# nsirons/DL-unet

Measured on AMD Instinct MI355X. Metric: 572x572 tiles/sec fwd+bwd, higher is better.
Workload: dtype f32; 1 GPU; batch=8/GPU 572x572x1 fwd+bwd+SGD fp32, 64-base-ch U-Net (BASELINE configs[1]); arithmetic=fp32 MFMA; 3x3 fwd/dgrad/wgrad as Winograd F(2x2,3x3), global_batch=8, tile=572, parallelism=dp1, loss=unweighted BCE-with-logits

## Files before the change

dl-unet_amd/csrc/wgradw.hip:

```cpp
#include "common.hpp"
#include "kernel_parts.hpp"
#include <cstdio>
#include <cstdlib>

namespace unet {

struct WgradWK {
    WgradP p;
    int TXn, TXg, TYn;
    int wy0, wx0;
    int NTg;
    int nsteps, steps_per;
    int ntile_i, ntile_j, nsplit;
    FastDiv d_spi, d_txg;
    size_t pstride;
    int xbytes, ybytes;
};

#ifndef WW_DBG
#define WW_DBG 0
#endif
constexpr int WW_PATCH = 32768, WW_EXTRA = 2048, WW_DY = 16384;
constexpr int WW_STAGE = WW_PATCH + WW_EXTRA + WW_DY;
constexpr int WW_NST = 3;
constexpr int WW_LDS = WW_NST * WW_STAGE;
constexpr int WW_SLAB = 9 * 64 * 64 + 64;

template <int N> __device__ __forceinline__ void ww_wait_vmcnt() { asm volatile("s_waitcnt vmcnt(%0)" ::"n"(N) : "memory"); }

__device__ __forceinline__ f32x2 wpk_add(f32x2 a, f32x2 b) { return a + b; }
__device__ __forceinline__ f32x2 wpk_sub(f32x2 a, f32x2 b) { return a - b; }

template <bool BUF>
__global__ __launch_bounds__(512, 1) void wgradw_f32_kernel(const WgradWK k)
{
    const WgradP &p = k.p;
    extern __shared__ __attribute__((aligned(16))) unsigned char smem[];

    const int tid = threadIdx.x, lane = tid & 63;
    const int wave = __builtin_amdgcn_readfirstlane(tid >> 6);
    const int wi = wave >> 1, wj = wave & 1;
    const int l15 = lane & 15, kg = lane >> 4;

    const int logical = xcd_slot();
    const int ntile = k.ntile_i * k.ntile_j;
    const int part = logical / ntile, tile = logical - part * ntile;
    const int it = tile / k.ntile_j, jt = tile - it * k.ntile_j;
    const int s0 = part * k.steps_per;
    int s1 = s0 + k.steps_per;
    s1 = s1 < k.nsteps ? s1 : k.nsteps;
    const int ns = s1 > s0 ? s1 - s0 : 0;

    const int d_cb = wave & 3, d_par = (wave >> 2) & 1;
    const int spi = k.TYn * k.TXg;

    const __amdgpu_buffer_rsrc_t rs_x = make_rsrc(p.X, BUF ? k.xbytes : 0);
    const __amdgpu_buffer_rsrc_t rs_y = make_rsrc(p.Y, BUF ? k.ybytes : 0);
    auto stage = [&](int buf, int step) {
        unsigned char *sb = smem + buf * WW_STAGE;
        int ln = lane;
        asm volatile("" : "+v"(ln));
        const int d_slot = ln >> 2, d_chunk = ln & 3;
        const int xch = p.xc0 + it * 64 + d_cb * 16 + d_chunk * 4;
        const int ych = p.yc0 + jt * 64 + d_cb * 16 + d_chunk * 4;
        const int Tb = step * 16;
        const bool tok = Tb + d_slot < k.NTg;
        const int img_b = fdiv(Tb, k.d_spi);
        const int rem_b = Tb - img_b * spi;
        const int ty_b = fdiv(rem_b, k.d_txg);
        int img = img_b, ty = ty_b, txg = rem_b - ty_b * k.TXg + d_slot;
        while (txg >= k.TXg) { txg -= k.TXg; ++ty; }
        while (ty >= k.TYn) { ty -= k.TYn; ++img; }
        img = img < p.NB ? img : p.NB - 1;
        {
            const int iy0 = (k.wy0 + 2 * ty + p.oy0) - p.xpad, ix = (k.wx0 + 2 * txg + p.ox0) - p.xpad + d_par;
            const bool xok = tok && (unsigned)ix < (unsigned)p.XW;
            const int base = ((img * p.XH + iy0) * p.XW + ix) * p.XC + xch;
#pragma unroll
            for (int qy = 0; qy < 4; ++qy) {
                const bool ok = xok && (unsigned)(iy0 + qy) < (unsigned)p.XH;
                unsigned char *dst = sb + ((qy * 2 + d_par) * 4 + d_cb) * 1024;
                if (BUF) {
                    lds_dma16(rs_x, dst, ok ? (base + qy * p.XW * p.XC) * 4 : LDS_DMA_OOB, 0);
                } else {
                    const float *g = ok ? p.X + (base + qy * p.XW * p.XC) : p.zeros;
                    GLDS16(g, dst);
                }
            }
        }
        {
            const int yy0 = k.wy0 + 2 * ty, xx = k.wx0 + 2 * txg + d_par;
            const bool xok = tok && txg < k.TXn && xx < p.YW;
            const int base = ((img * p.YH + yy0) * p.YW + xx) * p.YC + ych;
#pragma unroll
            for (int py = 0; py < 2; ++py) {
                const bool ok = xok && yy0 + py < p.YH;
                unsigned char *dst = sb + WW_PATCH + WW_EXTRA + ((py * 2 + d_par) * 4 + d_cb) * 1024;
                if (BUF) {
                    lds_dma16(rs_y, dst, ok ? (base + py * p.YW * p.YC) * 4 : LDS_DMA_OOB, 0);
                } else {
                    const float *g = ok ? p.Y + (base + py * p.YW * p.YC) : p.zeros;
                    GLDS16(g, dst);
                }
            }
        }
        if (wave < 2) {
            const int Te = step * 16 + 16;
            const bool eok = Te < k.NTg;
            const int Tec = eok ? Te : k.NTg - 1;
            const int eimg = fdiv(Tec, k.d_spi);
            const int erem = Tec - eimg * spi;
            const int ety = fdiv(erem, k.d_txg);
            const int etxg = erem - ety * k.TXg;
            const int e_row = (ln >> 4) + 4 * wave, e_cb = (ln >> 2) & 3;
            const int e_xch = p.xc0 + it * 64 + e_cb * 16 + d_chunk * 4;
            const int qy = e_row >> 1, par = e_row & 1;
            const int iy = (k.wy0 + 2 * ety + p.oy0) - p.xpad + qy, ix = (k.wx0 + 2 * etxg + p.ox0) - p.xpad + par;
            const bool ok = eok && (unsigned)iy < (unsigned)p.XH && (unsigned)ix < (unsigned)p.XW;
            const int eoff = ((eimg * p.XH + iy) * p.XW + ix) * p.XC + e_xch;
            if (BUF) {
                lds_dma16(rs_x, sb + WW_PATCH + wave * 1024, ok ? eoff * 4 : LDS_DMA_OOB, 0);
            } else {
                const float *g = ok ? p.X + eoff : p.zeros;
                GLDS16(g, sb + WW_PATCH + wave * 1024);
            }
        }
    };
    auto wait_landed = [&](bool one_in_flight) {
        if (!one_in_flight) ww_wait_vmcnt<0>();
        else if (wave < 2) ww_wait_vmcnt<7>();
        else ww_wait_vmcnt<6>();
    };

    f32x4 acc[16][2];
#pragma unroll
    for (int x = 0; x < 16; ++x)
#pragma unroll
        for (int j = 0; j < 2; ++j)
#pragma unroll
            for (int r = 0; r < 4; ++r) acc[x][j][r] = 0.f;
    f32x2 dbacc[2] = {{0.f, 0.f}, {0.f, 0.f}};

    const int a_base = wi * 1024 + l15 * 4;
    const int e_base = WW_PATCH + wi * 64 + l15 * 4;
    const bool last = kg == 3;
    const int y_base = WW_PATCH + WW_EXTRA + l15 * 4;

#define WW_SB() __builtin_amdgcn_sched_barrier(0)
    const int lv = a_base + kg * 64;
    const int lx = last ? e_base : lv + 9 * 64 + 256;
    const int lxs = last ? 512 : 8192;
    const int ly = y_base + 2 * wj * 1024 + kg * 64;
    auto v_read = [&](int buf, int pr, int j, f32x2 (&a)[4]) {
        if (WW_DBG & 4) { WW_SB(); return; }
        const unsigned char *pv = smem + buf * WW_STAGE + lv;
        if (j < 2 || pr == 0) {
#pragma unroll
            for (int qy = 0; qy < 4; ++qy) {
                const unsigned char *src = pv + ((2 * qy + (j & 1)) * 4096 + (8 * pr + (j >> 1)) * 64);
                a[qy][0] = *(const float *)(src);
                a[qy][1] = *(const float *)(src + 256);
            }
        } else {
            const unsigned char *px = smem + buf * WW_STAGE + lx + (j & 1) * (lxs >> 1);
#pragma unroll
            for (int qy = 0; qy < 4; ++qy) {
                a[qy][0] = *(const float *)(pv + ((2 * qy + (j & 1)) * 4096 + 9 * 64));
                a[qy][1] = *(const float *)(px + qy * lxs);
            }
        }
        WW_SB();
    };
    auto v_col = [&](int j, const f32x2 (&a)[4], f32x2 (&v)[16]) {
        if (WW_DBG & 8) { WW_SB(); return; }
        v[j] = wpk_sub(a[0], a[2]);
        v[4 + j] = wpk_add(a[1], a[2]);
        v[8 + j] = wpk_sub(a[2], a[1]);
        v[12 + j] = wpk_sub(a[1], a[3]);
        WW_SB();
    };
    auto v_row = [&](int i, f32x2 (&v)[16]) {
        if (WW_DBG & 8) { WW_SB(); return; }
        const f32x2 t0 = v[4 * i], t1 = v[4 * i + 1], t2 = v[4 * i + 2], t3 = v[4 * i + 3];
        v[4 * i + 0] = wpk_sub(t0, t2);
        v[4 * i + 1] = wpk_add(t1, t2);
        v[4 * i + 2] = wpk_sub(t2, t1);
        v[4 * i + 3] = wpk_sub(t1, t3);
        WW_SB();
    };
    auto z_read = [&](int buf, int pr, int c, f32x2 (&d)[4]) {
        if (WW_DBG & 4) { WW_SB(); return; }
        const unsigned char *ys = smem + buf * WW_STAGE + ly;
#pragma unroll
        for (int px = 0; px < 4; ++px) {
            d[px][0] = *(const float *)(ys + (px * 4096 + c * 1024 + pr * 512));
            d[px][1] = *(const float *)(ys + (px * 4096 + c * 1024 + pr * 512 + 256));
        }
        WW_SB();
    };
    auto group = [&](const f32x2 (&v)[16], const f32x2 (&d)[4], int c, bool RD, bool XF, int bufz, int prz, int cz, f32x2 (&dn)[4],
                     int bufv, int prv, f32x2 (&r)[4][4], f32x2 (&vn)[16]) {
        f32x2 zt[4];
        auto quad = [&](int b, int h) {
#pragma unroll
            for (int e = 0; e < 4; ++e)
                acc[4 * b + e][c] = __builtin_amdgcn_mfma_f32_16x16x4f32(v[4 * b + e][h], zt[e][h], acc[4 * b + e][c], 0, 0, 0);
            WW_SB();
        };
        zt[0] = d[0]; zt[1] = wpk_add(d[0], d[1]); zt[2] = wpk_sub(d[0], d[1]); zt[3] = d[1];
        WW_SB();
        quad(0, 0);
        z_read(bufz, prz, cz, dn);
        quad(0, 1);
        if (RD) v_read(bufv, prv, 0, r[0]);
        if (XF) { v_col(0, r[0], vn); v_col(1, r[1], vn); }
        zt[0] = wpk_add(d[0], d[2]); zt[3] = wpk_add(d[1], d[3]); zt[1] = wpk_add(zt[0], zt[3]); zt[2] = wpk_sub(zt[0], zt[3]);
        WW_SB();
        quad(1, 0);
        if (RD) v_read(bufv, prv, 1, r[1]);
        if (XF) { v_col(2, r[2], vn); v_col(3, r[3], vn); }
        quad(1, 1);
        if (RD) v_read(bufv, prv, 2, r[2]);
        if (XF) v_row(0, vn);
        zt[0] = wpk_sub(d[0], d[2]); zt[3] = wpk_sub(d[1], d[3]); zt[1] = wpk_add(zt[0], zt[3]); zt[2] = wpk_sub(zt[0], zt[3]);
        WW_SB();
        quad(2, 0);
        if (RD) v_read(bufv, prv, 3, r[3]);
        if (XF) v_row(1, vn);
        quad(2, 1);
        if (XF) v_row(2, vn);
        zt[0] = d[2]; zt[1] = wpk_add(d[2], d[3]); zt[2] = wpk_sub(d[2], d[3]); zt[3] = d[3];
        dbacc[c] = wpk_add(dbacc[c], wpk_add(wpk_add(d[0], d[1]), zt[1]));
        WW_SB();
        quad(3, 0);
        if (XF) {
            v_row(3, vn);
#pragma unroll
            for (int i = 0; i < 16; ++i) asm volatile("" : "+v"(vn[i]));
        }
        quad(3, 1);
    };
    if (ns > 0) {
        stage(0, s0);
        if (ns > 1) stage(1, s0 + 1);
        wait_landed(ns > 1);
        __builtin_amdgcn_s_barrier();
        const bool early = wave < 4;
        f32x2 va[16], vb[16], da[4], db_[4], r[4][4];
        {
#pragma unroll
            for (int j = 0; j < 4; ++j) { v_read(0, 0, j, r[j]); v_col(j, r[j], va); }
#pragma unroll
            for (int i = 0; i < 4; ++i) v_row(i, va);
        }
        z_read(0, 0, 0, da);
        for (int s = 0; s < ns; ++s) {
            const bool more = s + 2 < ns;
            const int buf = s % WW_NST, nbuf = (s + 1) % WW_NST;
            WW_SB();
            group(va, da, 0, true, false, buf, 0, 1, db_, buf, 1, r, vb);
            group(va, db_, 1, false, true, buf, 1, 0, da, buf, 1, r, vb);
            if (!(WW_DBG & 1)) ww_wait_vmcnt<0>();
            if (!(WW_DBG & 2)) __builtin_amdgcn_s_barrier();
            WW_SB();
            if (more && early && !(WW_DBG & 1)) stage((s + 2) % WW_NST, s0 + s + 2);
            WW_SB();
            group(vb, da, 0, true, false, buf, 1, 1, db_, nbuf, 0, r, va);
            group(vb, db_, 1, false, true, nbuf, 0, 0, da, nbuf, 0, r, va);
            if (more && !early && !(WW_DBG & 1)) stage((s + 2) % WW_NST, s0 + s + 2);
            WW_SB();
        }
    }
#undef WW_SB

    float *slab = p.slab + (size_t)(tile * k.nsplit + part) * k.pstride;
#pragma unroll
    for (int c = 0; c < 2; ++c) {
        f32x4 r[3][4];
#pragma unroll
        for (int b = 0; b < 4; ++b) {
            const f32x4 m0 = b == 3 ? -acc[b][c] : acc[b][c];
            const f32x4 m1 = b == 3 ? -acc[4 + b][c] : acc[4 + b][c];
            const f32x4 m2 = b == 3 ? -acc[8 + b][c] : acc[8 + b][c];
            const f32x4 m3 = b == 3 ? acc[12 + b][c] : -acc[12 + b][c];
            const f32x4 h = 0.5f * (m1 + m2);
            r[0][b] = m0 + h;
            r[1][b] = 0.5f * (m1 - m2);
            r[2][b] = h + m3;
        }
#pragma unroll
        for (int a = 0; a < 3; ++a) {
            const f32x4 h = 0.5f * (r[a][1] + r[a][2]);
            const f32x4 o0 = r[a][0] + h, o1 = 0.5f * (r[a][1] - r[a][2]), o2 = h + r[a][3];
            float *dst = slab + ((a * 3) * 64 + (2 * wj + c) * 16 + l15) * 64 + wi * 16 + 4 * kg;
            *(f32x4 *)(dst) = o0;
            *(f32x4 *)(dst + 4096) = o1;
            *(f32x4 *)(dst + 8192) = o2;
        }
    }
    if (wi == 0) {
#pragma unroll
        for (int c = 0; c < 2; ++c) {
            float v = dbacc[c][0] + dbacc[c][1];
            v += __shfl_xor(v, 16, 64);
            v += __shfl_xor(v, 32, 64);
            if (kg == 0) slab[9 * 64 * 64 + (2 * wj + c) * 16 + l15] = v;
        }
    }
}

template <int PG>
__global__ __launch_bounds__(64 * PG) void wgradw_reduce_kernel(const float *__restrict__ slab, int nsplit, size_t pstride, int ntile_j,
                                                            float *__restrict__ out, long si, long sj, long st,
                                                            float *__restrict__ db, int db_c0)
{
    const int tile = blockIdx.x >> 6, jb = blockIdx.x & 63;
    const int j = threadIdx.x & 63, grp = threadIdx.x >> 6;
    const float *src = slab + (size_t)tile * nsplit * pstride + (size_t)jb * 64 + j;
    float m[9];
#pragma unroll
    for (int x = 0; x < 9; ++x) m[x] = 0.f;
    for (int P = grp; P < nsplit; P += PG) {
        const float *s = src + (size_t)P * pstride;
#pragma unroll
        for (int x = 0; x < 9; ++x) m[x] += s[x * 4096];
    }
    __shared__ float red[PG][3][64];
#pragma unroll
    for (int xq = 0; xq < 3; ++xq) {
        if (xq) __syncthreads();
#pragma unroll
        for (int x = 0; x < 3; ++x) red[grp][x][j] = m[3 * xq + x];
        __syncthreads();
        if (grp == 0) {
#pragma unroll
            for (int x = 0; x < 3; ++x) {
                float v = red[0][x][j];
#pragma unroll
                for (int g = 1; g < PG; ++g) v += red[g][x][j];
                m[3 * xq + x] = v;
            }
        }
    }
    if (grp == 0) {
        const int it = tile / ntile_j, jt = tile - it * ntile_j;
        float *o = out + (size_t)(it * 64 + j) * si + (size_t)(jt * 64 + jb) * sj;
#pragma unroll
        for (int t = 0; t < 9; ++t) o[t * st] = m[t];
    }
    if (db && jb == 0 && (tile / ntile_j) == 0) {
        __syncthreads();
        const int jt = tile % ntile_j;
        float v = 0.f;
        for (int P = grp; P < nsplit; P += PG) v += slab[((size_t)tile * nsplit + P) * pstride + 9 * 64 * 64 + j];
        red[grp][0][j] = v;
        __syncthreads();
        if (grp == 0) {
            float t = red[0][0][j];
#pragma unroll
            for (int g = 1; g < PG; ++g) t += red[g][0][j];
            db[db_c0 + jt * 64 + j] = t;
        }
    }
}

bool wgradw_applicable(const WgradP &p)
{
    if (p.TY != 3 || p.TX != 3 || p.stride != 1) return false;
    if (p.Ci % 64 != 0 || p.Cj % 64 != 0 || p.db_on_x) return false;
    return true;
}

static void ww_decompose(const WgradP &p, WgradWK &k, int cus)
{
    k.p = p;
    k.wy0 = p.ywin0; k.wx0 = p.xwin0;
    k.TYn = cdiv(p.ywin1 - p.ywin0, 2);
    k.TXn = cdiv(p.xwin1 - p.xwin0, 2);
    k.TXg = k.TXn + 1;
    k.NTg = p.NB * k.TYn * k.TXg;
    k.nsteps = cdiv(k.NTg, 16);
    k.ntile_i = p.Ci / 64; k.ntile_j = p.Cj / 64;
    const int ntile = k.ntile_i * k.ntile_j;
    int nsplit = cus / ntile;
    if (nsplit < 1) nsplit = 1;
    if (nsplit > k.nsteps) nsplit = k.nsteps;
    k.nsplit = nsplit;
    k.steps_per = cdiv(k.nsteps, nsplit);
    k.d_spi = make_fastdiv((unsigned)(k.TYn * k.TXg));
    k.d_txg = make_fastdiv((unsigned)k.TXg);
    k.pstride = WW_SLAB;
}

size_t wgradw_slab_need(const WgradP &p)
{
    if (!wgradw_applicable(p)) return 0;
    WgradWK k;
    ww_decompose(p, k, 256);
    return (size_t)k.ntile_i * k.ntile_j * k.nsplit * k.pstride * sizeof(float);
}

int launch_wgradw(const WgradP &p, hipStream_t st)
{
    const size_t xb = tensor_bytes(p.NB, p.XH, p.XW, p.XC, sizeof(float)), yb = tensor_bytes(p.NB, p.YH, p.YW, p.YC, sizeof(float));
    const bool buf = get_lds_dma_mode() != 0 && fits_buffer(xb) && fits_buffer(yb);
    const auto launch = buf ? launch_profiled<wgradw_f32_kernel<true>, WgradWK> : launch_profiled<wgradw_f32_kernel<false>, WgradWK>;
    WgradWK k;
    int cus = device_cu_count();
    if (cus > 256) cus = 256;
    ww_decompose(p, k, cus);
    k.xbytes = buf ? (int)xb : 0; k.ybytes = buf ? (int)yb : 0;
    const int ntile = k.ntile_i * k.ntile_j;
    const size_t need = (size_t)ntile * k.nsplit * k.pstride * sizeof(float);
    ARG_CHECK(need <= p.slab_bytes, "wgradw: slab scratch too small (%zu < %zu)", p.slab_bytes, need);
    ARG_CHECK(tensor_elems(p.NB, p.XH, p.XW, p.XC) < LIMIT_31BIT && tensor_elems(p.NB, p.YH, p.YW, p.YC) < LIMIT_31BIT,
              "wgradw: tensor exceeds 31-bit element offsets");
    if (p.db) ARG_CHECK(p.ywin0 == 0 && p.xwin0 == 0 && p.ywin1 == p.YH && p.xwin1 == p.YW, "wgradw: fused bias gradient needs the full Y window");
    char tag[96];
    snprintf(tag, sizeof(tag), "wgradw<%d> Ci=%d Cj=%d Y=%dx%d tiles=%dx%d steps=%d split=%d", (int)buf, p.Ci, p.Cj, p.YH, p.YW, k.TYn, k.TXn, k.nsteps, k.nsplit);
    if (int rc_ = launch(ntile * k.nsplit, 512, WW_LDS, st, PK_WGRAD, tag, wgrad_alg_flops(p), 2.0 * k.nsteps * 16.0 * 16.0 * p.Ci * p.Cj, wgrad_alg_bytes(p), k)) return rc_;
    prof_begin(PK_REDUCE, "wgradw_reduce", st, 0.0, 0.0, (double)ntile * k.nsplit * k.pstride * 4.0 + 9.0 * p.Ci * p.Cj * 4.0);
    if (ntile <= 4 && k.nsplit >= 32)
        hipLaunchKernelGGL(wgradw_reduce_kernel<16>, dim3(ntile * 64), dim3(1024), 0, st, p.slab, k.nsplit, k.pstride, k.ntile_j,
                           p.out, p.si, p.sj, p.st, p.db, p.yc0);
    else
        hipLaunchKernelGGL(wgradw_reduce_kernel<4>, dim3(ntile * 64), dim3(256), 0, st, p.slab, k.nsplit, k.pstride, k.ntile_j,
                           p.out, p.si, p.sj, p.st, p.db, p.yc0);
    prof_end(st);
    HIP_TRY(hipGetLastError());
    return 0;
}

}
```

Measured before the change: 255.4 tiles/s.

## Repartition Winograd wgrad work across waves by transform row

Each wave now owns one Winograd transform row (A) for half of the input-channel blocks, across all four output-channel columns, rather than a wi/wj block across all 16 transform elements. This cuts per-wave input-transform work and LDS reads, since each wave only reads and transforms the rows it needs and skips unneeded dy loads. Per-wave accumulators are then shuffled through LDS in two phases to restore the old layout for the output transform. The cost is an extra LDS exchange with several barriers, a different MFMA/LDS interleave, and templated code paths per wave.

After: 257.7 tiles/s (median of 6 runs). Within noise of the previous version (+0.9%).

```diff
diff --git a/dl-unet_amd/csrc/wgradw.hip b/dl-unet_amd/csrc/wgradw.hip
--- a/dl-unet_amd/csrc/wgradw.hip
+++ b/dl-unet_amd/csrc/wgradw.hip
@@ -2,6 +2,7 @@
 #include "kernel_parts.hpp"
 #include <cstdio>
 #include <cstdlib>
+#include <type_traits>
 
 namespace unet {
 
@@ -39,7 +40,6 @@
 
     const int tid = threadIdx.x, lane = tid & 63;
     const int wave = __builtin_amdgcn_readfirstlane(tid >> 6);
-    const int wi = wave >> 1, wj = wave & 1;
     const int l15 = lane & 15, kg = lane >> 4;
 
     const int logical = xcd_slot();
@@ -132,17 +132,20 @@
         else ww_wait_vmcnt<6>();
     };
 
-    f32x4 acc[16][2];
-#pragma unroll
-    for (int x = 0; x < 16; ++x)
-#pragma unroll
-        for (int j = 0; j < 2; ++j)
-#pragma unroll
-            for (int r = 0; r < 4; ++r) acc[x][j][r] = 0.f;
+    const int h = wave >> 2, a = (wave & 3) ^ h;
+    f32x4 ar[2][4][4];
+#pragma unroll
+    for (int i = 0; i < 2; ++i)
+#pragma unroll
+        for (int c = 0; c < 4; ++c)
+#pragma unroll
+            for (int e = 0; e < 4; ++e)
+#pragma unroll
+                for (int r = 0; r < 4; ++r) ar[i][c][e][r] = 0.f;
     f32x2 dbacc[2] = {{0.f, 0.f}, {0.f, 0.f}};
 
-    const int a_base = wi * 1024 + l15 * 4;
-    const int e_base = WW_PATCH + wi * 64 + l15 * 4;
+    const int a_base = 2 * h * 1024 + l15 * 4;
+    const int e_base = WW_PATCH + 2 * h * 64 + l15 * 4;
     const bool last = kg == 3;
     const int y_base = WW_PATCH + WW_EXTRA + l15 * 4;
 
@@ -150,128 +153,161 @@
     const int lv = a_base + kg * 64;
     const int lx = last ? e_base : lv + 9 * 64 + 256;
     const int lxs = last ? 512 : 8192;
-    const int ly = y_base + 2 * wj * 1024 + kg * 64;
-    auto v_read = [&](int buf, int pr, int j, f32x2 (&a)[4]) {
-        if (WW_DBG & 4) { WW_SB(); return; }
-        const unsigned char *pv = smem + buf * WW_STAGE + lv;
-        if (j < 2 || pr == 0) {
-#pragma unroll
-            for (int qy = 0; qy < 4; ++qy) {
-                const unsigned char *src = pv + ((2 * qy + (j & 1)) * 4096 + (8 * pr + (j >> 1)) * 64);
-                a[qy][0] = *(const float *)(src);
-                a[qy][1] = *(const float *)(src + 256);
-            }
-        } else {
-            const unsigned char *px = smem + buf * WW_STAGE + lx + (j & 1) * (lxs >> 1);
-#pragma unroll
-            for (int qy = 0; qy < 4; ++qy) {
-                a[qy][0] = *(const float *)(pv + ((2 * qy + (j & 1)) * 4096 + 9 * 64));
-                a[qy][1] = *(const float *)(px + qy * lxs);
-            }
-        }
-        WW_SB();
-    };
-    auto v_col = [&](int j, const f32x2 (&a)[4], f32x2 (&v)[16]) {
-        if (WW_DBG & 8) { WW_SB(); return; }
-        v[j] = wpk_sub(a[0], a[2]);
-        v[4 + j] = wpk_add(a[1], a[2]);
-        v[8 + j] = wpk_sub(a[2], a[1]);
-        v[12 + j] = wpk_sub(a[1], a[3]);
-        WW_SB();
-    };
-    auto v_row = [&](int i, f32x2 (&v)[16]) {
-        if (WW_DBG & 8) { WW_SB(); return; }
-        const f32x2 t0 = v[4 * i], t1 = v[4 * i + 1], t2 = v[4 * i + 2], t3 = v[4 * i + 3];
-        v[4 * i + 0] = wpk_sub(t0, t2);
-        v[4 * i + 1] = wpk_add(t1, t2);
-        v[4 * i + 2] = wpk_sub(t2, t1);
-        v[4 * i + 3] = wpk_sub(t1, t3);
-        WW_SB();
-    };
-    auto z_read = [&](int buf, int pr, int c, f32x2 (&d)[4]) {
-        if (WW_DBG & 4) { WW_SB(); return; }
-        const unsigned char *ys = smem + buf * WW_STAGE + ly;
-#pragma unroll
-        for (int px = 0; px < 4; ++px) {
-            d[px][0] = *(const float *)(ys + (px * 4096 + c * 1024 + pr * 512));
-            d[px][1] = *(const float *)(ys + (px * 4096 + c * 1024 + pr * 512 + 256));
-        }
-        WW_SB();
-    };
-    auto group = [&](const f32x2 (&v)[16], const f32x2 (&d)[4], int c, bool RD, bool XF, int bufz, int prz, int cz, f32x2 (&dn)[4],
-                     int bufv, int prv, f32x2 (&r)[4][4], f32x2 (&vn)[16]) {
-        f32x2 zt[4];
-        auto quad = [&](int b, int h) {
-#pragma unroll
-            for (int e = 0; e < 4; ++e)
-                acc[4 * b + e][c] = __builtin_amdgcn_mfma_f32_16x16x4f32(v[4 * b + e][h], zt[e][h], acc[4 * b + e][c], 0, 0, 0);
-            WW_SB();
-        };
-        zt[0] = d[0]; zt[1] = wpk_add(d[0], d[1]); zt[2] = wpk_sub(d[0], d[1]); zt[3] = d[1];
-        WW_SB();
-        quad(0, 0);
-        z_read(bufz, prz, cz, dn);
-        quad(0, 1);
-        if (RD) v_read(bufv, prv, 0, r[0]);
-        if (XF) { v_col(0, r[0], vn); v_col(1, r[1], vn); }
-        zt[0] = wpk_add(d[0], d[2]); zt[3] = wpk_add(d[1], d[3]); zt[1] = wpk_add(zt[0], zt[3]); zt[2] = wpk_sub(zt[0], zt[3]);
-        WW_SB();
-        quad(1, 0);
-        if (RD) v_read(bufv, prv, 1, r[1]);
-        if (XF) { v_col(2, r[2], vn); v_col(3, r[3], vn); }
-        quad(1, 1);
-        if (RD) v_read(bufv, prv, 2, r[2]);
-        if (XF) v_row(0, vn);
-        zt[0] = wpk_sub(d[0], d[2]); zt[3] = wpk_sub(d[1], d[3]); zt[1] = wpk_add(zt[0], zt[3]); zt[2] = wpk_sub(zt[0], zt[3]);
-        WW_SB();
-        quad(2, 0);
-        if (RD) v_read(bufv, prv, 3, r[3]);
-        if (XF) v_row(1, vn);
-        quad(2, 1);
-        if (XF) v_row(2, vn);
-        zt[0] = d[2]; zt[1] = wpk_add(d[2], d[3]); zt[2] = wpk_sub(d[2], d[3]); zt[3] = d[3];
-        dbacc[c] = wpk_add(dbacc[c], wpk_add(wpk_add(d[0], d[1]), zt[1]));
-        WW_SB();
-        quad(3, 0);
-        if (XF) {
-            v_row(3, vn);
-#pragma unroll
-            for (int i = 0; i < 16; ++i) asm volatile("" : "+v"(vn[i]));
-        }
-        quad(3, 1);
+    const int lxi = last ? 64 : 1024;
+    const int ly = y_base + kg * 64;
+
+    auto kloop = [&](auto A_, auto BC_) {
+        constexpr int A = decltype(A_)::value, BC = decltype(BC_)::value;
+        constexpr int P = A == 0 ? 0 : A == 2 ? 2 : 1, Q = A == 3 ? 3 : A == 2 ? 1 : 2;
+        auto v_read1 = [&](int buf, int pr, int i, int j, f32x2 (&t)[2]) {
+            const unsigned char *pv = smem + buf * WW_STAGE + lv + i * 1024;
+            if (j < 2 || pr == 0) {
+#pragma unroll
+                for (int q = 0; q < 2; ++q) {
+                    const unsigned char *src = pv + ((2 * (q ? Q : P) + (j & 1)) * 4096 + (8 * pr + (j >> 1)) * 64);
+                    t[q][0] = *(const float *)(src);
+                    t[q][1] = *(const float *)(src + 256);
+                }
+            } else {
+                const unsigned char *px = smem + buf * WW_STAGE + lx + i * lxi + (j & 1) * (lxs >> 1);
+#pragma unroll
+                for (int q = 0; q < 2; ++q) {
+                    t[q][0] = *(const float *)(pv + ((2 * (q ? Q : P) + (j & 1)) * 4096 + 9 * 64));
+                    t[q][1] = *(const float *)(px + (q ? Q : P) * lxs);
+                }
+            }
+        };
+        auto v_read = [&](int buf, int pr, int i, int j, f32x2 (&r)[2][4][2]) {
+            if (WW_DBG & 4) { WW_SB(); return; }
+            v_read1(buf, pr, i, j, r[i][j]);
+            v_read1(buf, pr, i, j + 1, r[i][j + 1]);
+            WW_SB();
+        };
+        auto v_col = [&](const f32x2 (&r)[4][2], f32x2 (&t)[4]) {
+            if (WW_DBG & 8) { WW_SB(); return; }
+#pragma unroll
+            for (int j = 0; j < 4; ++j) t[j] = A == 1 ? wpk_add(r[j][0], r[j][1]) : wpk_sub(r[j][0], r[j][1]);
+            WW_SB();
+        };
+        auto v_row = [&](const f32x2 (&t)[4], f32x2 (&v)[4]) {
+            if (WW_DBG & 8) { WW_SB(); return; }
+            v[0] = wpk_sub(t[0], t[2]);
+            v[1] = wpk_add(t[1], t[2]);
+            v[2] = wpk_sub(t[2], t[1]);
+            v[3] = wpk_sub(t[1], t[3]);
+            WW_SB();
+        };
+        auto z_need = [&](int px, int c) { return px < 2 ? (A != 3 || c == BC || c == BC + 1) : A != 0; };
+        auto z_read = [&](int buf, int pr, int c, f32x2 (&d)[4]) {
+            if (WW_DBG & 4) { WW_SB(); return; }
+            const unsigned char *ys = smem + buf * WW_STAGE + ly;
+#pragma unroll
+            for (int px = 0; px < 4; ++px) {
+                if (!z_need(px, c)) continue;
+                d[px][0] = *(const float *)(ys + (px * 4096 + c * 1024 + pr * 512));
+                d[px][1] = *(const float *)(ys + (px * 4096 + c * 1024 + pr * 512 + 256));
+            }
+            WW_SB();
+        };
+        auto unit = [&](const f32x2 (&v)[2][4], const f32x2 (&d)[4], int c, int bufz, int prz, int cz, f32x2 (&dn)[4],
+                        int RD, int bufv, int prv, f32x2 (&r)[2][4][2], int XF, f32x2 (&vn)[2][4]) {
+            f32x2 zt[4], t[4];
+            auto quad = [&](int i, int hh) {
+#pragma unroll
+                for (int e = 0; e < 4; ++e)
+                    ar[i][c][e] = __builtin_amdgcn_mfma_f32_16x16x4f32(v[i][e][hh], zt[e][hh], ar[i][c][e], 0, 0, 0);
+                WW_SB();
+            };
+            if (A == 0) {
+                zt[0] = d[0]; zt[1] = wpk_add(d[0], d[1]); zt[2] = wpk_sub(d[0], d[1]); zt[3] = d[1];
+            } else if (A == 1) {
+                zt[0] = wpk_add(d[0], d[2]); zt[3] = wpk_add(d[1], d[3]); zt[1] = wpk_add(zt[0], zt[3]); zt[2] = wpk_sub(zt[0], zt[3]);
+            } else if (A == 2) {
+                zt[0] = wpk_sub(d[0], d[2]); zt[3] = wpk_sub(d[1], d[3]); zt[1] = wpk_add(zt[0], zt[3]); zt[2] = wpk_sub(zt[0], zt[3]);
+            } else {
+                zt[0] = d[2]; zt[1] = wpk_add(d[2], d[3]); zt[2] = wpk_sub(d[2], d[3]); zt[3] = d[3];
+                if (c == BC || c == BC + 1) dbacc[(c - BC) & 1] = wpk_add(dbacc[(c - BC) & 1], wpk_add(wpk_add(d[0], d[1]), zt[1]));
+            }
+            WW_SB();
+            quad(0, 0);
+            z_read(bufz, prz, cz, dn);
+            quad(1, 0);
+            if (RD >= 0) v_read(bufv, prv, RD, 0, r);
+            if (XF >= 0) v_col(r[XF], t);
+            quad(0, 1);
+            if (RD >= 0) v_read(bufv, prv, RD, 2, r);
+            if (XF >= 0) {
+                v_row(t, vn[XF]);
+#pragma unroll
+                for (int e = 0; e < 4; ++e) asm volatile("" : "+v"(vn[XF][e]));
+            }
+            quad(1, 1);
+        };
+        const bool early = wave < 4;
+        f32x2 va[2][4], vb[2][4], da[4], db_[4], r[2][4][2];
+#pragma unroll
+        for (int i = 0; i < 2; ++i) {
+            f32x2 t[4];
+            v_read(0, 0, i, 0, r);
+            v_read(0, 0, i, 2, r);
+            v_col(r[i], t);
+            v_row(t, va[i]);
+        }
+        z_read(0, 0, 0, da);
+        for (int s = 0; s < ns; ++s) {
+            const bool more = s + 2 < ns;
+            const int buf = s % WW_NST, nbuf = (s + 1) % WW_NST;
+            WW_SB();
+            unit(va, da, 0, buf, 0, 1, db_, 0, buf, 1, r, -1, vb);
+            unit(va, db_, 1, buf, 0, 2, da, 1, buf, 1, r, -1, vb);
+            unit(va, da, 2, buf, 0, 3, db_, -1, buf, 1, r, 0, vb);
+            unit(va, db_, 3, buf, 1, 0, da, -1, buf, 1, r, 1, vb);
+            if (!(WW_DBG & 1)) ww_wait_vmcnt<0>();
+            if (!(WW_DBG & 2)) __builtin_amdgcn_s_barrier();
+            WW_SB();
+            if (more && early && !(WW_DBG & 1)) stage((s + 2) % WW_NST, s0 + s + 2);
+            WW_SB();
+            unit(vb, da, 0, buf, 1, 1, db_, 0, nbuf, 0, r, -1, va);
+            unit(vb, db_, 1, buf, 1, 2, da, 1, nbuf, 0, r, -1, va);
+            unit(vb, da, 2, buf, 1, 3, db_, -1, nbuf, 0, r, 0, va);
+            unit(vb, db_, 3, nbuf, 0, 0, da, -1, nbuf, 0, r, 1, va);
+            if (more && !early && !(WW_DBG & 1)) stage((s + 2) % WW_NST, s0 + s + 2);
+            WW_SB();
+        }
     };
     if (ns > 0) {
         stage(0, s0);
         if (ns > 1) stage(1, s0 + 1);
         wait_landed(ns > 1);
         __builtin_amdgcn_s_barrier();
-        const bool early = wave < 4;
-        f32x2 va[16], vb[16], da[4], db_[4], r[4][4];
-        {
-#pragma unroll
-            for (int j = 0; j < 4; ++j) { v_read(0, 0, j, r[j]); v_col(j, r[j], va); }
-#pragma unroll
-            for (int i = 0; i < 4; ++i) v_row(i, va);
-        }
-        z_read(0, 0, 0, da);
-        for (int s = 0; s < ns; ++s) {
-            const bool more = s + 2 < ns;
-            const int buf = s % WW_NST, nbuf = (s + 1) % WW_NST;
-            WW_SB();
-            group(va, da, 0, true, false, buf, 0, 1, db_, buf, 1, r, vb);
-            group(va, db_, 1, false, true, buf, 1, 0, da, buf, 1, r, vb);
-            if (!(WW_DBG & 1)) ww_wait_vmcnt<0>();
-            if (!(WW_DBG & 2)) __builtin_amdgcn_s_barrier();
-            WW_SB();
-            if (more && early && !(WW_DBG & 1)) stage((s + 2) % WW_NST, s0 + s + 2);
-            WW_SB();
-            group(vb, da, 0, true, false, buf, 1, 1, db_, nbuf, 0, r, va);
-            group(vb, db_, 1, false, true, nbuf, 0, 0, da, nbuf, 0, r, va);
-            if (more && !early && !(WW_DBG & 1)) stage((s + 2) % WW_NST, s0 + s + 2);
-            WW_SB();
-        }
+        using std::integral_constant;
+        if (a == 0) kloop(integral_constant<int, 0>(), integral_constant<int, -2>());
+        else if (a == 1) kloop(integral_constant<int, 1>(), integral_constant<int, -2>());
+        else if (a == 2) kloop(integral_constant<int, 2>(), integral_constant<int, -2>());
+        else if (h == 0) kloop(integral_constant<int, 3>(), integral_constant<int, 0>());
+        else kloop(integral_constant<int, 3>(), integral_constant<int, 2>());
     }
 #undef WW_SB
+
+    const int wi = wave >> 1, wj = wave & 1;
+    f32x4 acc[16][2];
+    {
+        f32x4 *tl = (f32x4 *)smem + lane;
+        __syncthreads();
+        if (h == 1) { __syncthreads(); __syncthreads(); }
+#pragma unroll
+        for (int i = 0; i < 2; ++i)
+#pragma unroll
+            for (int c = 0; c < 4; ++c)
+#pragma unroll
+                for (int e = 0; e < 4; ++e) tl[(((4 * a + e) * 2 + i) * 4 + c) * 64] = ar[i][c][e];
+        __syncthreads();
+#pragma unroll
+        for (int x = 0; x < 16; ++x)
+#pragma unroll
+            for (int c = 0; c < 2; ++c) acc[x][c] = tl[((x * 2 + (wi & 1)) * 4 + 2 * wj + c) * 64];
+        if (h == 0) { __syncthreads(); __syncthreads(); }
+    }
 
     float *slab = p.slab + (size_t)(tile * k.nsplit + part) * k.pstride;
 #pragma unroll
@@ -298,13 +334,13 @@
             *(f32x4 *)(dst + 8192) = o2;
         }
     }
-    if (wi == 0) {
+    if (a == 3) {
 #pragma unroll
         for (int c = 0; c < 2; ++c) {
             float v = dbacc[c][0] + dbacc[c][1];
             v += __shfl_xor(v, 16, 64);
             v += __shfl_xor(v, 32, 64);
-            if (kg == 0) slab[9 * 64 * 64 + (2 * wj + c) * 16 + l15] = v;
+            if (kg == 0) slab[9 * 64 * 64 + (2 * h + c) * 16 + l15] = v;
         }
     }
 }
```
